# bentotten/radiation_ppo

Measured on AMD Instinct MI355X. Metric: env steps/sec (whole node) at 4096 envs; PPO iters/sec at 1/2/4/8 GPUs, higher is better.
Workload: dtype f32 policy / f64+int32 env

## Files before the change

include/radsearch.h:

```cpp
#ifndef RADSEARCH_H
#define RADSEARCH_H

#include <stddef.h>
#include <stdint.h>

#ifdef __cplusplus
extern "C" {
#endif

#define RS_ABI_VERSION 4
#define RS_OBS_DIM 11
#define RS_NUM_ACTIONS 9
#define RS_MAX_AGENTS 8
#define RS_MAX_OBS 7

typedef void* rs_stream_t;
typedef struct rs_handle rs_handle;

enum {
    RS_OK = 0,
    RS_ERR_INVALID_ARG = 1,
    RS_ERR_HIP = 2,
    RS_ERR_WORKSPACE = 3,
    RS_ERR_UNSUPPORTED = 4
// ... 127 lines not shown
typedef struct rs_update_state {
    int32_t adam_step;
    int32_t stopped;
    int32_t iters;
    int32_t pad;
    double last_stats[5];
} rs_update_state;

int rs_adam_step(const rs_mlp_params* actor, const rs_mlp_params* critic, const float* grads, float* m, float* v,
                 const double* stats, rs_update_state* state, float lr, float kl_threshold, rs_stream_t stream);

int rs_ppo_update_step(const rs_mlp_params* actor, const rs_mlp_params* critic, const rs_ppo_batch* batch, float* grads,
                       double* stats, void* workspace, float* m, float* v, rs_update_state* state, float lr, float kl_threshold,
                       rs_stream_t stream);

typedef struct rs_maps rs_maps;
enum {
    RS_MAPERR_RING_FULL = 1,
    RS_MAPERR_VISIT_OVERFLOW = 2,
    RS_MAPERR_OFF_MAP = 4
};
size_t rs_maps_state_bytes(int32_t num_envs, int32_t num_agents, int32_t steps_per_episode, int32_t map_x, int32_t map_y);
int rs_maps_create(int32_t num_envs, int32_t num_agents, int32_t steps_per_episode, int32_t map_x, int32_t map_y,
                   double resolution_accuracy, const float* visit_table, void* workspace, size_t workspace_bytes,
                   rs_stream_t stream, rs_maps** out);
void rs_maps_destroy(rs_maps* m);
int rs_maps_reset(rs_maps* m, const uint8_t* mask, rs_stream_t stream);
int rs_maps_update(rs_maps* m, rs_handle* env, const float* obs, const float* pred, const uint8_t* mask, rs_stream_t stream);
int rs_maps_stack(rs_maps* m, float* actor_stack, float* critic_stack, rs_stream_t stream);
int rs_maps_field(rs_maps* m, const char* name, void** dev_ptr, int32_t* elem_bytes, int32_t* rows, int32_t* cols);
// ... 274 lines not shown
```

radiation_ppo_amd/_lib.py:

```python
import ctypes as C
import os

import torch

_PKG = os.path.dirname(os.path.abspath(__file__))
LIB_PATH = os.environ.get("RS_LIB_PATH") or os.path.join(_PKG, "lib", "librs_hip.so")

RS_OBS_DIM = 11
RS_MAX_AGENTS = 8
RS_MAX_OBS = 7

ENVERR_ZERO_DIST = 1
ENVERR_IDLE_STALL = 2
ENVERR_CORRECT_CAP = 4
ENVERR_BAD_ACTION = 8
ENVERR_NO_PATH = 16

MAPERR_RING_FULL = 1
MAPERR_VISIT_OVERFLOW = 2
MAPERR_OFF_MAP = 4


class RsConfig(C.Structure):
    _fields_ = [
# ... 78 lines not shown
                                   C.c_void_p, C.c_void_p, C.c_void_p]),
    ("rs_error_flags", C.c_int, [C.c_void_p, C.c_void_p, C.POINTER(C.c_uint32)]),
    ("rs_policy_forward", C.c_int, [C.POINTER(RsMlpParams), C.POINTER(RsMlpParams), C.c_void_p, C.c_int32, C.c_void_p,
                                    C.c_void_p, C.c_void_p]),
    ("rs_ff_team_step", C.c_int, [C.POINTER(RsMlpParams), C.POINTER(RsMlpParams), C.c_int32, C.c_void_p, C.c_void_p, C.c_void_p,
                                  C.c_void_p, C.c_void_p, C.c_void_p, C.c_int32, C.c_void_p]),
    ("rs_rollout", C.c_int, [C.c_void_p, C.POINTER(RsMlpParams), C.POINTER(RsMlpParams), C.POINTER(RsRolloutArgs), C.c_void_p]),
    ("rs_rollout_lds_bytes", C.c_size_t, [C.c_int]),
    ("rs_ppo_grad_workspace_bytes", C.c_size_t, []),
    ("rs_ppo_grad", C.c_int, [C.POINTER(RsMlpParams), C.POINTER(RsMlpParams), C.POINTER(RsPpoBatch), C.c_void_p, C.c_void_p,
                              C.c_void_p, C.c_void_p, C.c_void_p]),
    ("rs_adam_step", C.c_int, [C.POINTER(RsMlpParams), C.POINTER(RsMlpParams), C.c_void_p, C.c_void_p, C.c_void_p, C.c_void_p,
                               C.c_void_p, C.c_float, C.c_float, C.c_void_p]),
    ("rs_ppo_update_step", C.c_int, [C.POINTER(RsMlpParams), C.POINTER(RsMlpParams), C.POINTER(RsPpoBatch), C.c_void_p, C.c_void_p,
                                     C.c_void_p, C.c_void_p, C.c_void_p, C.c_void_p, C.c_float, C.c_float, C.c_void_p]),
    ("rs_maps_state_bytes", C.c_size_t, [C.c_int32, C.c_int32, C.c_int32, C.c_int32, C.c_int32]),
    ("rs_maps_create", C.c_int, [C.c_int32, C.c_int32, C.c_int32, C.c_int32, C.c_int32, C.c_double, C.c_void_p, C.c_void_p,
                                 C.c_size_t, C.c_void_p, C.POINTER(C.c_void_p)]),
    ("rs_maps_destroy", None, [C.c_void_p]),
    ("rs_maps_reset", C.c_int, [C.c_void_p, C.c_void_p, C.c_void_p]),
    ("rs_maps_update", C.c_int, [C.c_void_p, C.c_void_p, C.c_void_p, C.c_void_p, C.c_void_p, C.c_void_p]),
    ("rs_maps_stack", C.c_int, [C.c_void_p, C.c_void_p, C.c_void_p, C.c_void_p]),
    ("rs_maps_field", C.c_int, [C.c_void_p, C.c_char_p, C.POINTER(C.c_void_p), C.POINTER(C.c_int32), C.POINTER(C.c_int32),
                                C.POINTER(C.c_int32)]),
    ("rs_cnn_trunk_slab_row", C.c_int32, [C.c_int32]),
    ("rs_cnn_trunk_slab_rows", C.c_int32, [C.c_int64, C.c_int32]),
    ("rs_cnn_trunk_forward_grid", C.c_int32, [C.c_int64, C.c_int32]),
    ("rs_cnn_trunk_scratch_floats", C.c_int32, [C.c_int32]),
    ("rs_cnn_trunk_forward", C.c_int, [C.c_void_p, C.c_void_p, C.c_void_p, C.c_int32, C.c_int32, C.c_int64, C.c_void_p, C.c_void_p,
                                       C.c_void_p, C.c_void_p, C.c_void_p, C.c_void_p, C.c_void_p, C.c_void_p, C.c_void_p, C.c_void_p]),
# ... 141 lines not shown
```

radiation_ppo_amd/build.py:

```python
import os
import shutil
import subprocess
import sys
from concurrent.futures import ThreadPoolExecutor

PKG = os.path.dirname(os.path.abspath(__file__))
ROOT = os.path.dirname(PKG)
CSRC = os.path.join(PKG, "csrc")
LIBDIR = os.path.join(PKG, "lib")
OBJDIR = os.path.join(LIBDIR, "obj")
LIB = os.path.join(LIBDIR, "librs_hip.so")

SOURCES = ["rs_env.hip", "rs_ppo.hip", "rs_maps.hip", "rs_cnn.hip", "rs_cnn_sized.hip", "rs_pfgru.hip", "rs_gru.hip", "rs_pfgru_train.hip", "rs_rnn_policy.hip", "rs_welford.hip", "rs_cnn_loss.hip",
           "rs_rnn_sized.hip", "rs_pfgru_sized.hip", "rs_pfgru_sized_train.hip", "rs_ff_team.hip", "rs_eval.hip", "rs_draws.hip", "rs_cnn_eval.hip"]
CFLAGS = ["--offload-arch=gfx950", "-O3", "-std=c++17", "-fPIC", "-ffp-contract=off", "-fno-fast-math", "-Wall",
          "-Wno-unused-function"]
EXTRA_CFLAGS = {"rs_ppo.hip": ["-fno-slp-vectorize"], "rs_ff_team.hip": ["-fno-slp-vectorize"], "rs_eval.hip": ["-fno-slp-vectorize"],
                "rs_rnn_sized.hip": ["-mllvm", "-pragma-unroll-threshold=1000000"],
                "rs_pfgru_sized.hip": ["-mllvm", "-pragma-unroll-threshold=1000000"]}


def hipcc() -> str:
    for c in (os.environ.get("HIPCC"), shutil.which("hipcc"), "/opt/rocm/bin/hipcc"):
        if c and os.path.exists(c):
# ... 35 lines not shown
        cpus = os.cpu_count() or 1
    jobs = max(1, min(len(SOURCES), cpus, int(os.environ.get("MAX_JOBS") or cpus)))
    order = sorted(SOURCES, key=lambda f: f not in ("rs_rnn_sized.hip", "rs_pfgru_sized.hip"))
    with ThreadPoolExecutor(max_workers=jobs) as ex:
        done = dict(zip(order, ex.map(compile_one, order)))
    objs = [done[f] for f in SOURCES]
    cmd = [cc, "--offload-arch=gfx950", "-shared", "-fPIC"] + objs + ["-o", lib]
    if verbose:
        print("[radiation_ppo_amd.build]", " ".join(cmd), flush=True)
    subprocess.run(cmd, check=True)
    return lib


if __name__ == "__main__":
    prio = sys.argv[sys.argv.index("--prio") + 1] if "--prio" in sys.argv else None
    if "--stamps" in sys.argv:
        build(force="--force" in sys.argv, defines=["RS_K7_STAMPS"], suffix="_stamps")
    elif "--skew" in sys.argv or prio is not None:
        skew = "--skew" in sys.argv
        build(force="--force" in sys.argv, defines=(["RS_K7_SKEW"] if skew else []) + ([f"RS_K7_PRIO={int(prio)}"] if prio is not None else []),
              suffix=("_skew" if skew else "") + (f"_prio{int(prio)}" if prio is not None else ""))
    else:
        build(force="--force" in sys.argv)
```

radiation_ppo_amd/csrc/rs_ppo.hip:

```cpp
#include <hip/hip_runtime.h>
#include <stdint.h>
#include <stdlib.h>
#include <string.h>

#include "../../include/radsearch.h"
#include "rs_mlp.hpp"
#include "rs_handle.hpp"

static inline RsMlpParams to_dev(const rs_mlp_params* p) { return RsMlpParams{p->w1, p->b1, p->w2, p->b2, p->w3, p->b3}; }

__device__ __forceinline__ void rs_exchange_x(const float (&xo)[RS_IN_PAD], float (&xp)[RS_IN_PAD]) {
#pragma unroll
    for (int k = 0; k < RS_IN_PAD; ++k) xp[k] = __shfl_xor(xo[k], 32);
}

__global__ void __launch_bounds__(64) rs_policy_forward_kernel(RsMlpParams pa, RsMlpParams pc, const float* __restrict__ x, int M,
                                                               float* __restrict__ logits, float* __restrict__ value) {
    extern __shared__ __align__(16) float smem_f[];
    RsMlpLds<8> A; RsMlpLds<1> Cn;
    A.carve(smem_f);
    Cn.carve(smem_f + rs_mlp_lds_floats(8));
    A.fill(pa); Cn.fill(pc);
    __syncthreads();
    const int lane = threadIdx.x & 63;
// ... 265 lines not shown

struct RsGradWs { float *pa, *pc; double *sa, *sc; int* snap; };

static RsGradWs rs_grad_ws(void* workspace) {
    const int slabs = RS_GRAD_BLOCKS;
    RsGradWs w;
    w.pa = static_cast<float*>(workspace);
    w.pc = w.pa + (size_t)slabs * rs_net_params(8);
    w.sa = reinterpret_cast<double*>((reinterpret_cast<uintptr_t>(w.pc + (size_t)slabs * rs_net_params(1)) + 255) & ~uintptr_t(255));
    w.sc = w.sa + (size_t)slabs * 5;
    w.snap = reinterpret_cast<int*>(w.sc + (size_t)slabs * 5);
    return w;
}

static int rs_launch_k7(const rs_mlp_params* actor, const rs_mlp_params* critic, const rs_ppo_batch* batch, const RsGradWs& w,
                        const int32_t* stop_flag, const rs_update_state* ust, hipStream_t s, bool pair = false) {
    const size_t lds_a = sizeof(float) * (size_t)rs_grad2_lds_floats(8);
    const size_t lds_c = sizeof(float) * (size_t)rs_grad2_lds_floats(1);
    const size_t lds_p = lds_a > lds_c ? lds_a : lds_c;
    if (pair) {
        if (hipFuncSetAttribute(reinterpret_cast<const void*>(rs_ppo_grad2_pair_kernel), hipFuncAttributeMaxDynamicSharedMemorySize, (int)lds_p) != hipSuccess)
            return RS_ERR_HIP;
    } else if (hipFuncSetAttribute(reinterpret_cast<const void*>(rs_ppo_grad2_kernel<8>), hipFuncAttributeMaxDynamicSharedMemorySize, (int)lds_a) != hipSuccess ||
               hipFuncSetAttribute(reinterpret_cast<const void*>(rs_ppo_grad2_kernel<1>), hipFuncAttributeMaxDynamicSharedMemorySize, (int)lds_c) != hipSuccess)
        return RS_ERR_HIP;
    int threads = 512;
#if defined(RS_K7_STAMPS) || defined(RS_K7_SKEW)
    if (const char* e = getenv("RS_K7_THREADS")) threads = atoi(e) == 256 ? 256 : 512;
#endif
    if (pair) {
        hipLaunchKernelGGL(rs_ppo_grad2_pair_kernel, dim3(2 * RS_GRAD_BLOCKS), dim3(threads), lds_p, s, to_dev(actor), to_dev(critic), *batch,
                           w.pa, w.pc, w.sa, w.sc, stop_flag, ust, ust ? w.snap : (int*)nullptr);
        return RS_OK;
    }
    hipLaunchKernelGGL(rs_ppo_grad2_kernel<8>, dim3(RS_GRAD_BLOCKS), dim3(threads), lds_a, s, to_dev(actor), *batch, w.pa, w.sa, stop_flag,
                       (const rs_update_state*)nullptr, (int*)nullptr);
    hipLaunchKernelGGL(rs_ppo_grad2_kernel<1>, dim3(RS_GRAD_BLOCKS), dim3(threads), lds_c, s, to_dev(critic), *batch, w.pc, w.sc, stop_flag,
                       ust, ust ? w.snap : (int*)nullptr);
    return RS_OK;
}

int rs_ppo_grad(const rs_mlp_params* actor, const rs_mlp_params* critic, const rs_ppo_batch* batch, float* grads,
                double* stats, void* workspace, const int32_t* stop_flag, rs_stream_t stream) {
    if (!actor || !critic || !batch || !grads || !stats || !workspace || batch->M < 1) return RS_ERR_INVALID_ARG;
    if (reinterpret_cast<uintptr_t>(workspace) & 255u) return RS_ERR_WORKSPACE;
    hipStream_t s = static_cast<hipStream_t>(stream);
    const RsGradWs w = rs_grad_ws(workspace);
    if (const int rc = rs_launch_k7(actor, critic, batch, w, stop_flag, nullptr, s)) return rc;
    const int np = rs_net_params(8) + rs_net_params(1);
    hipLaunchKernelGGL(rs_ppo_reduce_kernel, dim3((np + 63) / 64), dim3(1024), 0, s, w.pa, w.pc, w.sa, w.sc, RS_GRAD_BLOCKS, grads, stats,
                       batch->alpha, batch->vf_coef, stop_flag);
    return hipGetLastError() == hipSuccess ? RS_OK : RS_ERR_HIP;
}

int rs_ppo_update_step(const rs_mlp_params* actor, const rs_mlp_params* critic, const rs_ppo_batch* batch, float* grads,
                       double* stats, void* workspace, float* m, float* v, rs_update_state* state, float lr, float kl_threshold,
                       rs_stream_t stream) {
    if (!actor || !critic || !batch || !grads || !stats || !workspace || !m || !v || !state || batch->M < 1) return RS_ERR_INVALID_ARG;
    if (reinterpret_cast<uintptr_t>(workspace) & 255u) return RS_ERR_WORKSPACE;
    hipStream_t s = static_cast<hipStream_t>(stream);
    const RsGradWs w = rs_grad_ws(workspace);
    const char* split = getenv("RS_PPO_SPLIT_GRAD");
    if (const int rc = rs_launch_k7(actor, critic, batch, w, &state->stopped, state, s, !(split && *split && *split != '0'))) return rc;
    const int np = rs_net_params(8) + rs_net_params(1);
    hipLaunchKernelGGL(rs_ppo_tail_kernel, dim3((np + 63) / 64), dim3(1024), 0, s, w.pa, w.pc, w.sa, w.sc, RS_GRAD_BLOCKS, grads, stats,
                       batch->alpha, batch->vf_coef, rs_param_seg(actor, critic), m, v, state, w.snap, lr, kl_threshold);
    return hipGetLastError() == hipSuccess ? RS_OK : RS_ERR_HIP;
}

#ifdef RS_K7_STAMPS
int rs_debug_k7_stamps(unsigned long long* out, int clear) {
    if (hipDeviceSynchronize() != hipSuccess) return RS_ERR_HIP;
    if (out && hipMemcpyFromSymbol(out, HIP_SYMBOL(rs_k7_stamp_table), sizeof(unsigned long long) * 2 * RS_K7_NPH) != hipSuccess) return RS_ERR_HIP;
    if (clear) {
        unsigned long long z[2 * RS_K7_NPH] = {0};
        if (hipMemcpyToSymbol(HIP_SYMBOL(rs_k7_stamp_table), z, sizeof(z)) != hipSuccess) return RS_ERR_HIP;
    }
    return RS_OK;
}
#endif

#ifdef RS_K7_SKEW
// ... 36 lines not shown
```

radiation_ppo_amd/csrc/rs_ppo_grad2.hpp:

```cpp
#pragma once
#include "rs_mlp.hpp"

#define RS_T2 33

#ifdef RS_K7_STAMPS
#define RS_K7_NPH 16
__device__ unsigned long long rs_k7_stamp_table[2][RS_K7_NPH];
#define RS_STAMP_ENTRY const unsigned long long st_rt0 = __builtin_amdgcn_s_memrealtime(); const unsigned long long st_t0 = rs_k7_now();
#define RS_STAMP_DECL unsigned long long st_acc[RS_K7_NPH] = {0}; unsigned long long st_last = rs_k7_now(); st_acc[12] = st_last - st_t0;
#define RS_STAMP_EXIT(net) do { RS_STAMP(13); if ((threadIdx.x & 63) == 0) { st_acc[14] = __builtin_amdgcn_s_memrealtime() - st_rt0; \
                           for (int q = 0; q < RS_K7_NPH; ++q) atomicAdd(&rs_k7_stamp_table[net][q], st_acc[q]); } } while (0)
#define RS_STAMP(i) do { __builtin_amdgcn_sched_barrier(0); asm volatile("; RS_STAMP_MARK " #i); const unsigned long long t_ = rs_k7_now(); st_acc[i] += t_ - st_last; st_last = t_; \
                         __builtin_amdgcn_sched_barrier(0); } while (0)
__device__ __forceinline__ unsigned long long rs_k7_now() {
    unsigned long long t;
    asm volatile("s_memtime %0\n\ts_waitcnt lgkmcnt(0)" : "=s"(t) :: "memory");
    return t;
}
#else
#define RS_STAMP_ENTRY
#define RS_STAMP_DECL
#define RS_STAMP_EXIT(net)
#ifdef RS_K7_NO_PHASE_FENCE
#define RS_STAMP(i) do {} while (0)
// ... 31 lines not shown
#define RS_SKEW_RELEASED
#define RS_SKEW_PAIRS(net, slots)
#define RS_SKEW_EXIT(net)
#endif

#ifndef RS_K7_PRIO
#define RS_K7_PRIO 1
#endif
#ifndef RS_K7_PRIO_BIT
#define RS_K7_PRIO_BIT 15
#endif
#define RS_K7_PROG_FLOATS 8

#define RS_XRAW 400
#define RS_XSC 192
#define RS_G2_WAVE_FLOATS ((64 + 32) * RS_T2 + RS_XRAW + RS_XSC + 64)

__host__ __device__ constexpr int rs_grad2_lds_floats(int nout) {
    return ((rs_mlp_lds_floats(nout) + 3) & ~3) + 2 * 2 * 16 * 64 + 2 * 4 * 64 + 8 * RS_G2_WAVE_FLOATS + RS_K7_PROG_FLOATS + RS_SKEW_LDS_FLOATS;
}

__device__ __forceinline__ float rs_other_half(float x, int h) {
    const auto r = __builtin_amdgcn_permlane32_swap(__float_as_uint(x), __float_as_uint(x), false, false);
    return __uint_as_float(h ? r[0] : r[1]);
}

typedef float rs_f2 __attribute__((ext_vector_type(2)));

__device__ __forceinline__ void rs_tanh_scaled16(f32x16& v) {
#pragma unroll
    for (int r = 0; r < 16; r += 2) {
        const rs_f2 e = (rs_f2){1.0f, 1.0f} + (rs_f2){__builtin_amdgcn_exp2f(v[r]), __builtin_amdgcn_exp2f(v[r + 1])};
        const rs_f2 t = __builtin_elementwise_fma((rs_f2){-2.0f, -2.0f}, (rs_f2){__builtin_amdgcn_rcpf(e.x), __builtin_amdgcn_rcpf(e.y)},
                                                  (rs_f2){1.0f, 1.0f});
        v[r] = t.x; v[r + 1] = t.y;
    }
}

__device__ __forceinline__ rs_f2 rs_dtanh2(rs_f2 d, rs_f2 hv) { return __builtin_elementwise_fma(-(d * hv), hv, d); }

__device__ __forceinline__ void rs_stage32(float* T, const f32x16& v, int c, int h) {
#pragma unroll
    for (int r = 0; r < 16; ++r) T[rs_kappa(r, h) * RS_T2 + c] = v[r];
}

template <int NOUT>
__device__ __forceinline__ void rs_ppo_grad2_body(const RsMlpParams prm, const rs_ppo_batch B, float* partial,
                                                  double* stat_partial, const int* stop,
                                                  const rs_update_state* ust, int* snap,
                                                  const int bid, const int nblocks) {
    extern __shared__ __align__(16) float smem_f[];
    if (snap && bid == 0 && threadIdx.x == 0) { snap[0] = ust->adam_step; snap[1] = ust->stopped; }
    if (stop && *stop) return;
    RS_STAMP_ENTRY
    RS_SKEW_ENTRY
    RsMlpLds<NOUT> W;
    W.carve(smem_f);
    float* w2tf = smem_f + ((rs_mlp_lds_floats(NOUT) + 3) & ~3);
    float* w3tf = w2tf + 2 * 2 * 16 * 64;
    const int wid = __builtin_amdgcn_readfirstlane(threadIdx.x >> 6);
    const int lane = threadIdx.x & 63, h = lane >> 5, c = lane & 31;
    const int l15 = lane & 15, l4 = lane >> 4;
    float* Qt = w3tf + 2 * 4 * 64 + wid * RS_G2_WAVE_FLOATS;
    float* Pt = Qt + 64 * RS_T2;
    float* xraw = Pt + 32 * RS_T2;
// ... 42 lines not shown
#pragma unroll
        for (int r = 0; r < 16; ++r) { acc2[a][0][r] = 0.f; acc2[a][1][r] = 0.f; }
#pragma unroll
    for (int r = 0; r < 4; ++r) {
#pragma unroll
        for (int a = 0; a < 4; ++a) acc1[a][r] = 0.f;
        acc3[0][r] = 0.f; acc3[1][r] = 0.f;
    }
    f32x4 accs;
#pragma unroll
    for (int r = 0; r < 4; ++r) accs[r] = 0.f;

    const int trips = (groups + n_waves - 1) / n_waves;
    const long x_last = (long)M * RS_IN - 1;
    auto dma_rows = [&](int g) {
        const char* gx = reinterpret_cast<const char*>(B.x + (long)g * (32 * RS_IN));
        const int lim = (int)(x_last - (long)g * (32 * RS_IN));
#pragma unroll
        for (int i = 0; i < 6; ++i) {
            const int o = min(i * 64 + lane, lim);
            __builtin_amdgcn_global_load_lds((const __attribute__((address_space(1))) void*)(gx + 4u * (unsigned)o),
                                             (__attribute__((address_space(3))) void*)(xraw + i * 64), 4, 0, 0);
        }
    };
    auto dma_scal = [&](int g) {
        const int m0 = g * 32;
        const int ms = min(m0 + c, M - 1);
        if constexpr (NOUT == 8) {
            const int mi = min(m0 + (lane >> 1), M - 1);
            const int* src = reinterpret_cast<const int*>(B.act) + 2 * (size_t)mi + (lane & 1);
            __builtin_amdgcn_global_load_lds((const __attribute__((address_space(1))) void*)src,
                                             (__attribute__((address_space(3))) void*)(xsc), 4, 0, 0);
        }
        if constexpr (NOUT == 8) {
            const float* src = (h ? B.logp_old : B.adv) + ms;
            __builtin_amdgcn_global_load_lds((const __attribute__((address_space(1))) void*)src,
                                             (__attribute__((address_space(3))) void*)(xsc + 64), 4, 0, 0);
        }
        {
            const float* src = (h ? B.ret : B.w) + ms;
// ... 25 lines not shown
        const int bit = (int)(__builtin_amdgcn_readfirstlane((int)(__builtin_amdgcn_s_memtime() >> RS_K7_PRIO_BIT)) & 1) ^ (wid >> 2);
        if (bit) __builtin_amdgcn_s_setprio(1);
        else __builtin_amdgcn_s_setprio(0);
#endif
    };
#if RS_K7_PRIO == 4
    if (wid >= 4) __builtin_amdgcn_s_setprio(1);
#endif
    RS_STAMP_DECL
    for (int trip = 0; trip < trips; ++trip) {
        RS_STAMP(15);
        balance(RS_K7_PRIO == 2 ? 2 * trip : trip);
        const int gi_raw = wave_g + trip * n_waves;
        const int gi = gi_raw < groups ? gi_raw : groups - 1;
        const int m = gi * 32 + c;
        const bool valid = gi_raw < groups && m < M;
        asm volatile("s_waitcnt vmcnt(0)" ::: "memory");
#if defined(RS_K7_ALIGN) && RS_K7_ALIGN >= 1
        __builtin_amdgcn_s_barrier();
#endif
        const float wi = valid ? xsc[128 + c] : 0.0f;
        const int s_act = reinterpret_cast<const int*>(xsc)[2 * c];
        const float s_adv = xsc[64 + c], s_lpo = xsc[96 + c], s_ret = xsc[160 + c];
        float xv[6];
#pragma unroll
        for (int s6 = 0; s6 < 6; ++s6) xv[s6] = xraw[c * RS_IN + 2 * s6 + h];
        if (h) xv[5] = 1.0f;
        RS_STAMP(0);
        f32x16 H1[2], H2[2];
#pragma unroll
        for (int it = 0; it < 2; ++it)
#pragma unroll
            for (int r = 0; r < 16; ++r) H1[it][r] = 0.0f;
        {
            float a0 = w1b[(0 * 6 + 0) * 64 + lane], a1 = w1b[(1 * 6 + 0) * 64 + lane];
#pragma unroll
            for (int s = 0; s < 6; ++s) {
                const float b = xv[s];
                float n0 = 0.f, n1 = 0.f;
                if (s + 1 < 6) { n0 = w1b[(0 * 6 + s + 1) * 64 + lane]; n1 = w1b[(1 * 6 + s + 1) * 64 + lane]; }
                H1[0] = __builtin_amdgcn_mfma_f32_32x32x2f32(a0, b, H1[0], 0, 0, 0);
                H1[1] = __builtin_amdgcn_mfma_f32_32x32x2f32(a1, b, H1[1], 0, 0, 0);
// ... 187 lines not shown
                    acc3[hf] = __builtin_amdgcn_mfma_f32_4x4x1f32(av[q].z, bv[q].z, acc3[hf], 0, 0, 0);
                    accs = __builtin_amdgcn_mfma_f32_4x4x1f32(z1, 1.0f, accs, 0, 0, 0);
                    acc3[hf] = __builtin_amdgcn_mfma_f32_4x4x1f32(av[q].w, bv[q].w, acc3[hf], 0, 0, 0);
                }
            }
        }
        RS_STAMP(7);
        if (NOUT == 8) {
#pragma unroll
            for (int it = 0; it < 2; ++it) {
                f32x16 t;
#pragma unroll
                for (int r = 0; r < 16; ++r) t[r] = 0.f;
#pragma unroll
                for (int s = 0; s < 4; ++s) {
                    const float b = h ? dz[(2 * s + 1) % NOUT] : dz[(2 * s) % NOUT];
                    t = __builtin_amdgcn_mfma_f32_32x32x2f32(w3tf[(it * 4 + s) * 64 + lane], b, t, 0, 0, 0);
                }
#pragma unroll
                for (int r = 0; r < 16; r += 2) {
                    const rs_f2 d = rs_dtanh2((rs_f2){t[r], t[r + 1]}, (rs_f2){H2[it][r], H2[it][r + 1]});
                    H2[it][r] = d.x; H2[it][r + 1] = d.y;
                }
            }
        } else {
#pragma unroll
            for (int kt = 0; kt < 2; ++kt)
#pragma unroll
                for (int r = 0; r < 16; r += 2) {
                    const rs_f2 d = (rs_f2){w3v[kt * 16 + r], w3v[kt * 16 + r + 1]} * (rs_f2){dz[0], dz[0]};
                    const rs_f2 e = rs_dtanh2(d, (rs_f2){H2[kt][r], H2[kt][r + 1]});
// ... 29 lines not shown
                    n0 = wq[((0 * 2 + ((g4 + 1) >> 2)) * 4 + ((g4 + 1) & 3)) * 64];
                    n1 = wq[((1 * 2 + ((g4 + 1) >> 2)) * 4 + ((g4 + 1) & 3)) * 64];
                }
                D1[0] = __builtin_amdgcn_mfma_f32_32x32x2f32(a0.x, H2[kt][r0 + 0], D1[0], 0, 0, 0);
                D1[1] = __builtin_amdgcn_mfma_f32_32x32x2f32(a1.x, H2[kt][r0 + 0], D1[1], 0, 0, 0);
                D1[0] = __builtin_amdgcn_mfma_f32_32x32x2f32(a0.y, H2[kt][r0 + 1], D1[0], 0, 0, 0);
                D1[1] = __builtin_amdgcn_mfma_f32_32x32x2f32(a1.y, H2[kt][r0 + 1], D1[1], 0, 0, 0);
                D1[0] = __builtin_amdgcn_mfma_f32_32x32x2f32(a0.z, H2[kt][r0 + 2], D1[0], 0, 0, 0);
                D1[1] = __builtin_amdgcn_mfma_f32_32x32x2f32(a1.z, H2[kt][r0 + 2], D1[1], 0, 0, 0);
                D1[0] = __builtin_amdgcn_mfma_f32_32x32x2f32(a0.w, H2[kt][r0 + 3], D1[0], 0, 0, 0);
                D1[1] = __builtin_amdgcn_mfma_f32_32x32x2f32(a1.w, H2[kt][r0 + 3], D1[1], 0, 0, 0);
                a0 = n0; a1 = n1;
            }
        }
        float xb[8];
        {
            int gi_late = gi;
            asm volatile("" : "+v"(gi_late));
#pragma unroll
            for (int s8 = 0; s8 < 8; ++s8) {
                int n = gi_late * 32 + 4 * s8 + l4;
                n = n < M ? n : M - 1;
                xb[s8] = (l15 < RS_IN) ? B.x[(size_t)n * RS_IN + l15] : ((l15 == RS_IN) ? 1.0f : 0.0f);
            }
        }
#pragma unroll
        for (int it = 0; it < 2; ++it)
#pragma unroll
            for (int r = 0; r < 16; r += 2) {
                const rs_f2 hv = {Qt[(32 * it + rs_kappa(r, h)) * RS_T2 + c], Qt[(32 * it + rs_kappa(r + 1, h)) * RS_T2 + c]};
                const rs_f2 d = rs_dtanh2((rs_f2){D1[it][r], D1[it][r + 1]}, hv);
// ... 144 lines not shown
template <int NOUT>
__global__ void __launch_bounds__(512, 2) rs_ppo_grad2_kernel(RsMlpParams prm, rs_ppo_batch B, float* __restrict__ partial,
                                                              double* __restrict__ stat_partial, const int* __restrict__ stop,
                                                              const rs_update_state* __restrict__ ust, int* __restrict__ snap) {
    rs_ppo_grad2_body<NOUT>(prm, B, partial, stat_partial, stop, ust, snap, blockIdx.x, gridDim.x);
}

__global__ void __launch_bounds__(512, 2) rs_ppo_grad2_pair_kernel(RsMlpParams pa, RsMlpParams pc, rs_ppo_batch B, float* __restrict__ partial_a,
                                                                   float* __restrict__ partial_c, double* __restrict__ stat_a,
                                                                   double* __restrict__ stat_c, const int* __restrict__ stop,
                                                                   const rs_update_state* __restrict__ ust, int* __restrict__ snap) {
    const int G = gridDim.x >> 1;
    if ((int)blockIdx.x < G) rs_ppo_grad2_body<8>(pa, B, partial_a, stat_a, stop, nullptr, nullptr, blockIdx.x, G);
    else rs_ppo_grad2_body<1>(pc, B, partial_c, stat_c, stop, ust, snap, blockIdx.x - G, G);
}
```

radiation_ppo_amd/ppo.py:

```python
import ctypes as C
import os
from dataclasses import dataclass
from typing import Any, Dict, List, Optional

import torch
import torch.distributed as dist
import torch.nn as nn

from . import _lib
from .envs import RadSearchVec, gae as rs_gae_call


class FFActorCritic(nn.Module):

    def __init__(self, state_dim: int = 11, action_dim: int = 8, hidden: int = 64):
        super().__init__()
        self.actor = nn.Sequential(nn.Linear(state_dim, hidden), nn.Tanh(), nn.Linear(hidden, hidden), nn.Tanh(),
                                   nn.Linear(hidden, action_dim), nn.Softmax(dim=-1))
        self.critic = nn.Sequential(nn.Linear(state_dim, hidden), nn.Tanh(), nn.Linear(hidden, hidden), nn.Tanh(),
                                    nn.Linear(hidden, 1))

    def logits(self, x: torch.Tensor) -> torch.Tensor:
        for layer in list(self.actor)[:-1]:
            x = layer(x)
# ... 48 lines not shown
        self.lib = _lib.load()
        self.ac = ac
        dev = next(ac.parameters()).device
        self.bucket = torch.zeros(N_PARAMS + 16, dtype=torch.float32, device=dev)
        self.grads = self.bucket[:N_PARAMS]
        self.stats = torch.zeros(5, dtype=torch.float64, device=dev)
        self.stats_from_bucket = False
        self.ws = torch.empty(self.lib.rs_ppo_grad_workspace_bytes() + 256, dtype=torch.uint8, device=dev)
        self._ws_ptr = self.ws.data_ptr() + (-self.ws.data_ptr()) % 256
        order = [ac.actor[0].weight, ac.actor[0].bias, ac.actor[2].weight, ac.actor[2].bias, ac.actor[4].weight, ac.actor[4].bias,
                 ac.critic[0].weight, ac.critic[0].bias, ac.critic[2].weight, ac.critic[2].bias, ac.critic[4].weight, ac.critic[4].bias]
        self.m = torch.zeros(N_PARAMS, dtype=torch.float32, device=dev)
        self.v = torch.zeros(N_PARAMS, dtype=torch.float32, device=dev)
        self.state = torch.zeros(8, dtype=torch.float64, device=dev)
        self.state_i32 = self.state.view(torch.int32)
        self.views = []
        o = 0
        for p in order:
            self.views.append((p, self.grads[o:o + p.numel()].view_as(p)))
            o += p.numel()
        assert o == N_PARAMS

    def begin_update(self) -> None:
        self.state_i32[1:3].zero_()

    def adam_step(self, lr: float, kl_threshold: float) -> None:
        import ctypes as C
        pa, pc = mlp_params(self.ac.actor), mlp_params(self.ac.critic)
        _lib.check(self.lib.rs_adam_step(C.byref(pa), C.byref(pc), self.bucket.data_ptr(), self.m.data_ptr(), self.v.data_ptr(),
                                         None if self.stats_from_bucket else self.stats.data_ptr(), self.state.data_ptr(), lr, kl_threshold,
# ... 17 lines not shown
        with _lib.timed("rs_ppo_grad"):
            _lib.check(self.lib.rs_ppo_grad(C.byref(pa), C.byref(pc), C.byref(b), self.bucket.data_ptr(), self.stats.data_ptr(),
                                            self._ws_ptr, (self.state.data_ptr() + 4) if use_stop_flag else None,
                                            torch.cuda.current_stream(X.device).cuda_stream), "rs_ppo_grad")
        return self.stats, self.grads

    def bind(self, X, act, adv, ret, logp_old, w, clip_ratio: float, alpha: float, vf_coef: float = 0.01) -> None:
        import ctypes as C
        for t in (X, adv, ret, logp_old, w):
            assert t.dtype == torch.float32 and t.is_contiguous()
        assert act.dtype == torch.int64 and act.is_contiguous()
        b = _lib.RsPpoBatch(X.data_ptr(), act.data_ptr(), adv.data_ptr(), ret.data_ptr(), logp_old.data_ptr(), w.data_ptr(),
                            X.shape[0], clip_ratio, alpha, vf_coef)
        pa, pc = mlp_params(self.ac.actor), mlp_params(self.ac.critic)
        self._bound = (b, pa, pc, (X, act, adv, ret, logp_old, w))
        self._bound_args = (C.byref(pa), C.byref(pc), C.byref(b), self.bucket.data_ptr(), self.stats.data_ptr(), self._ws_ptr,
                            self.m.data_ptr(), self.v.data_ptr(), self.state.data_ptr())
        self._bound_dev = X.device

    def step_bound(self, lr: float, kl_threshold: float):
        self.stats_from_bucket = False
        with _lib.timed("rs_ppo_grad"):
            _lib.check(self.lib.rs_ppo_update_step(*self._bound_args, lr, kl_threshold,
                                                   torch.cuda.current_stream(self._bound_dev).cuda_stream), "rs_ppo_update_step")
        return self.stats, self.grads

    def step(self, X, act, adv, ret, logp_old, w, clip_ratio: float, alpha: float, vf_coef: float = 0.01, *, lr: float,
             kl_threshold: float):
        self.bind(X, act, adv, ret, logp_old, w, clip_ratio, alpha, vf_coef)
        return self.step_bound(lr, kl_threshold)

    def allreduce(self) -> None:
        Collectives.all_reduce_sum(self.bucket)
        self.stats_from_bucket = True

    def assign_grads(self) -> None:
        for p, g in self.views:
            p.grad = g

# ... 279 lines not shown
            else:
                kl_reached = True
            kk += 1
        self.pi_scheduler.step()
        return UpdateResult(stop_iteration=kk, loss_policy=last[4], loss_critic=last[3], loss_predictor=0.0,
                            kl_divergence=last[0], Entropy=last[1], ClipFrac=last[2], LocLoss=0.0)

    def _update_agent_fused(self, X, act, adv, ret, logp_old, w) -> UpdateResult:
        if self._fused is None:
            self._fused = FusedPPOGrad(self.agent)
        f = self._fused
        lr = self.actor_learning_rate * (0.99 ** (self.epochs_done // 100))
        thr = 1.5 * self.target_kl
        f.begin_update()
        one_rank = _world() == 1 and not os.environ.get("RS_PPO_SPLIT_TAIL")
        if one_rank:
            f.bind(X, act, adv, ret, logp_old, w, self.clip_ratio, self.alpha)
        for _ in range(self.train_pi_iters):
            if one_rank:
                f.step_bound(lr, thr)
                continue
            stats, grads = f(X, act, adv, ret, logp_old, w, self.clip_ratio, self.alpha, use_stop_flag=True)
            if _world() > 1:
                f.allreduce()
            f.adam_step(lr, thr)
        kk, stopped, _, last = f.read_state()
        self.epochs_done += 1
        return UpdateResult(stop_iteration=kk, loss_policy=last[4], loss_critic=last[3], loss_predictor=0.0,
                            kl_divergence=last[0], Entropy=last[1], ClipFrac=last[2], LocLoss=0.0)

    def save(self, path: str) -> None:
        torch.save(self.agent.state_dict(), path)

    def load(self, path: str) -> None:
        self.agent.load_state_dict(torch.load(path, map_location=self.device, weights_only=True))

    def resume_state(self) -> Dict[str, Any]:
# ... 480 lines not shown
```

Measured before the change: 44.93 million.

## Prebuild swizzled PPO batch image once per update for direct LDS DMA loads

Adds a kernel that repacks the PPO batch (observations, actions, advantages, returns, logp, weights) into a per-32-row record laid out in the exact lane order the gradient kernel consumes. The gradient kernels get image variants that load these records with whole-wave global_load_lds DMA pieces and float4 loads, in place of per-row strided gathers with bounds clamping. The image is built once per bind and reused across all train_pi_iters. The multi-rank path now also binds once instead of rebuilding args every iteration. The cost is an extra buffer and a build kernel per update, plus a compile-time parts mask that selects which sections use the image.

```diff
diff --git a/include/radsearch.h b/include/radsearch.h
--- a/include/radsearch.h
+++ b/include/radsearch.h
@@ -165,6 +165,14 @@
                        double* stats, void* workspace, float* m, float* v, rs_update_state* state, float lr, float kl_threshold,
                        rs_stream_t stream);
 
+size_t rs_ppo_batch_image_bytes(int32_t M);
+int rs_ppo_batch_image_build(const rs_ppo_batch* batch, void* image, rs_stream_t stream);
+int rs_ppo_grad_img(const rs_mlp_params* actor, const rs_mlp_params* critic, const rs_ppo_batch* batch, const void* image, float* grads,
+                    double* stats, void* workspace, const int32_t* stop_flag, rs_stream_t stream);
+int rs_ppo_update_step_img(const rs_mlp_params* actor, const rs_mlp_params* critic, const rs_ppo_batch* batch, const void* image,
+                           float* grads, double* stats, void* workspace, float* m, float* v, rs_update_state* state, float lr,
+                           float kl_threshold, rs_stream_t stream);
+
 typedef struct rs_maps rs_maps;
 enum {
     RS_MAPERR_RING_FULL = 1,
diff --git a/radiation_ppo_amd/_lib.py b/radiation_ppo_amd/_lib.py
--- a/radiation_ppo_amd/_lib.py
+++ b/radiation_ppo_amd/_lib.py
@@ -116,6 +116,12 @@
                                C.c_void_p, C.c_float, C.c_float, C.c_void_p]),
     ("rs_ppo_update_step", C.c_int, [C.POINTER(RsMlpParams), C.POINTER(RsMlpParams), C.POINTER(RsPpoBatch), C.c_void_p, C.c_void_p,
                                      C.c_void_p, C.c_void_p, C.c_void_p, C.c_void_p, C.c_float, C.c_float, C.c_void_p]),
+    ("rs_ppo_batch_image_bytes", C.c_size_t, [C.c_int32]),
+    ("rs_ppo_batch_image_build", C.c_int, [C.POINTER(RsPpoBatch), C.c_void_p, C.c_void_p]),
+    ("rs_ppo_grad_img", C.c_int, [C.POINTER(RsMlpParams), C.POINTER(RsMlpParams), C.POINTER(RsPpoBatch), C.c_void_p, C.c_void_p, C.c_void_p,
+                                  C.c_void_p, C.c_void_p, C.c_void_p]),
+    ("rs_ppo_update_step_img", C.c_int, [C.POINTER(RsMlpParams), C.POINTER(RsMlpParams), C.POINTER(RsPpoBatch), C.c_void_p, C.c_void_p,
+                                         C.c_void_p, C.c_void_p, C.c_void_p, C.c_void_p, C.c_void_p, C.c_float, C.c_float, C.c_void_p]),
     ("rs_maps_state_bytes", C.c_size_t, [C.c_int32, C.c_int32, C.c_int32, C.c_int32, C.c_int32]),
     ("rs_maps_create", C.c_int, [C.c_int32, C.c_int32, C.c_int32, C.c_int32, C.c_int32, C.c_double, C.c_void_p, C.c_void_p,
                                  C.c_size_t, C.c_void_p, C.POINTER(C.c_void_p)]),
diff --git a/radiation_ppo_amd/build.py b/radiation_ppo_amd/build.py
--- a/radiation_ppo_amd/build.py
+++ b/radiation_ppo_amd/build.py
@@ -73,7 +73,12 @@
 
 if __name__ == "__main__":
     prio = sys.argv[sys.argv.index("--prio") + 1] if "--prio" in sys.argv else None
-    if "--stamps" in sys.argv:
+    parts = sys.argv[sys.argv.index("--img-parts") + 1] if "--img-parts" in sys.argv else None
+    if parts is not None:
+        st = "--stamps" in sys.argv
+        build(force="--force" in sys.argv, defines=(["RS_K7_STAMPS"] if st else []) + [f"RS_K7_IMG_PARTS={int(parts)}"],
+              suffix=("_stamps" if st else "") + f"_img{int(parts)}")
+    elif "--stamps" in sys.argv:
         build(force="--force" in sys.argv, defines=["RS_K7_STAMPS"], suffix="_stamps")
     elif "--skew" in sys.argv or prio is not None:
         skew = "--skew" in sys.argv
diff --git a/radiation_ppo_amd/csrc/rs_ppo.hip b/radiation_ppo_amd/csrc/rs_ppo.hip
--- a/radiation_ppo_amd/csrc/rs_ppo.hip
+++ b/radiation_ppo_amd/csrc/rs_ppo.hip
@@ -303,11 +303,18 @@
 }
 
 static int rs_launch_k7(const rs_mlp_params* actor, const rs_mlp_params* critic, const rs_ppo_batch* batch, const RsGradWs& w,
-                        const int32_t* stop_flag, const rs_update_state* ust, hipStream_t s, bool pair = false) {
+                        const int32_t* stop_flag, const rs_update_state* ust, hipStream_t s, bool pair = false, const float* img = nullptr) {
     const size_t lds_a = sizeof(float) * (size_t)rs_grad2_lds_floats(8);
     const size_t lds_c = sizeof(float) * (size_t)rs_grad2_lds_floats(1);
     const size_t lds_p = lds_a > lds_c ? lds_a : lds_c;
-    if (pair) {
+    if (img) {
+        if (pair) {
+            if (hipFuncSetAttribute(reinterpret_cast<const void*>(rs_ppo_grad2_img_pair_kernel), hipFuncAttributeMaxDynamicSharedMemorySize, (int)lds_p) != hipSuccess)
+                return RS_ERR_HIP;
+        } else if (hipFuncSetAttribute(reinterpret_cast<const void*>(rs_ppo_grad2_img_kernel<8>), hipFuncAttributeMaxDynamicSharedMemorySize, (int)lds_a) != hipSuccess ||
+                   hipFuncSetAttribute(reinterpret_cast<const void*>(rs_ppo_grad2_img_kernel<1>), hipFuncAttributeMaxDynamicSharedMemorySize, (int)lds_c) != hipSuccess)
+            return RS_ERR_HIP;
+    } else if (pair) {
         if (hipFuncSetAttribute(reinterpret_cast<const void*>(rs_ppo_grad2_pair_kernel), hipFuncAttributeMaxDynamicSharedMemorySize, (int)lds_p) != hipSuccess)
             return RS_ERR_HIP;
     } else if (hipFuncSetAttribute(reinterpret_cast<const void*>(rs_ppo_grad2_kernel<8>), hipFuncAttributeMaxDynamicSharedMemorySize, (int)lds_a) != hipSuccess ||
@@ -317,6 +324,19 @@
 #if defined(RS_K7_STAMPS) || defined(RS_K7_SKEW)
     if (const char* e = getenv("RS_K7_THREADS")) threads = atoi(e) == 256 ? 256 : 512;
 #endif
+    int* const snap = ust ? w.snap : (int*)nullptr;
+    if (img) {
+        if (pair) {
+            hipLaunchKernelGGL(rs_ppo_grad2_img_pair_kernel, dim3(2 * RS_GRAD_BLOCKS), dim3(threads), lds_p, s, to_dev(actor), to_dev(critic), *batch,
+                               img, w.pa, w.pc, w.sa, w.sc, stop_flag, ust, snap);
+            return RS_OK;
+        }
+        hipLaunchKernelGGL(rs_ppo_grad2_img_kernel<8>, dim3(RS_GRAD_BLOCKS), dim3(threads), lds_a, s, to_dev(actor), *batch, img, w.pa, w.sa,
+                           stop_flag, (const rs_update_state*)nullptr, (int*)nullptr);
+        hipLaunchKernelGGL(rs_ppo_grad2_img_kernel<1>, dim3(RS_GRAD_BLOCKS), dim3(threads), lds_c, s, to_dev(critic), *batch, img, w.pc, w.sc,
+                           stop_flag, ust, snap);
+        return RS_OK;
+    }
     if (pair) {
         hipLaunchKernelGGL(rs_ppo_grad2_pair_kernel, dim3(2 * RS_GRAD_BLOCKS), dim3(threads), lds_p, s, to_dev(actor), to_dev(critic), *batch,
                            w.pa, w.pc, w.sa, w.sc, stop_flag, ust, ust ? w.snap : (int*)nullptr);
@@ -329,32 +349,70 @@
     return RS_OK;
 }
 
-int rs_ppo_grad(const rs_mlp_params* actor, const rs_mlp_params* critic, const rs_ppo_batch* batch, float* grads,
-                double* stats, void* workspace, const int32_t* stop_flag, rs_stream_t stream) {
+size_t rs_ppo_batch_image_bytes(int32_t M) {
+    return M < 1 ? 0 : (size_t)((M + 31) / 32) * RS_IMG_REC * sizeof(float);
+}
+
+int rs_ppo_batch_image_build(const rs_ppo_batch* batch, void* image, rs_stream_t stream) {
+    if (!batch || !image || batch->M < 1 || !batch->x || !batch->act || !batch->adv || !batch->ret || !batch->logp_old || !batch->w)
+        return RS_ERR_INVALID_ARG;
+    if (reinterpret_cast<uintptr_t>(image) & 15u) return RS_ERR_INVALID_ARG;
+    hipLaunchKernelGGL(rs_ppo_batch_image_kernel, dim3((batch->M + 31) / 32), dim3(256), 0, static_cast<hipStream_t>(stream), *batch,
+                       static_cast<float*>(image));
+    return hipGetLastError() == hipSuccess ? RS_OK : RS_ERR_HIP;
+}
+
+static int rs_ppo_grad_on(const rs_mlp_params* actor, const rs_mlp_params* critic, const rs_ppo_batch* batch, const float* image, float* grads,
+                          double* stats, void* workspace, const int32_t* stop_flag, rs_stream_t stream) {
     if (!actor || !critic || !batch || !grads || !stats || !workspace || batch->M < 1) return RS_ERR_INVALID_ARG;
     if (reinterpret_cast<uintptr_t>(workspace) & 255u) return RS_ERR_WORKSPACE;
     hipStream_t s = static_cast<hipStream_t>(stream);
     const RsGradWs w = rs_grad_ws(workspace);
-    if (const int rc = rs_launch_k7(actor, critic, batch, w, stop_flag, nullptr, s)) return rc;
+    if (const int rc = rs_launch_k7(actor, critic, batch, w, stop_flag, nullptr, s, false, image)) return rc;
     const int np = rs_net_params(8) + rs_net_params(1);
     hipLaunchKernelGGL(rs_ppo_reduce_kernel, dim3((np + 63) / 64), dim3(1024), 0, s, w.pa, w.pc, w.sa, w.sc, RS_GRAD_BLOCKS, grads, stats,
                        batch->alpha, batch->vf_coef, stop_flag);
     return hipGetLastError() == hipSuccess ? RS_OK : RS_ERR_HIP;
 }
 
-int rs_ppo_update_step(const rs_mlp_params* actor, const rs_mlp_params* critic, const rs_ppo_batch* batch, float* grads,
-                       double* stats, void* workspace, float* m, float* v, rs_update_state* state, float lr, float kl_threshold,
-                       rs_stream_t stream) {
+int rs_ppo_grad(const rs_mlp_params* actor, const rs_mlp_params* critic, const rs_ppo_batch* batch, float* grads,
+                double* stats, void* workspace, const int32_t* stop_flag, rs_stream_t stream) {
+    return rs_ppo_grad_on(actor, critic, batch, nullptr, grads, stats, workspace, stop_flag, stream);
+}
+
+int rs_ppo_grad_img(const rs_mlp_params* actor, const rs_mlp_params* critic, const rs_ppo_batch* batch, const void* image, float* grads,
+                    double* stats, void* workspace, const int32_t* stop_flag, rs_stream_t stream) {
+    if (!image || (reinterpret_cast<uintptr_t>(image) & 15u)) return RS_ERR_INVALID_ARG;
+    return rs_ppo_grad_on(actor, critic, batch, static_cast<const float*>(image), grads, stats, workspace, stop_flag, stream);
+}
+
+static int rs_ppo_update_step_on(const rs_mlp_params* actor, const rs_mlp_params* critic, const rs_ppo_batch* batch, const float* image,
+                                 float* grads, double* stats, void* workspace, float* m, float* v, rs_update_state* state, float lr,
+                                 float kl_threshold, rs_stream_t stream) {
     if (!actor || !critic || !batch || !grads || !stats || !workspace || !m || !v || !state || batch->M < 1) return RS_ERR_INVALID_ARG;
     if (reinterpret_cast<uintptr_t>(workspace) & 255u) return RS_ERR_WORKSPACE;
     hipStream_t s = static_cast<hipStream_t>(stream);
     const RsGradWs w = rs_grad_ws(workspace);
     const char* split = getenv("RS_PPO_SPLIT_GRAD");
-    if (const int rc = rs_launch_k7(actor, critic, batch, w, &state->stopped, state, s, !(split && *split && *split != '0'))) return rc;
+    if (const int rc = rs_launch_k7(actor, critic, batch, w, &state->stopped, state, s, !(split && *split && *split != '0'), image)) return rc;
     const int np = rs_net_params(8) + rs_net_params(1);
     hipLaunchKernelGGL(rs_ppo_tail_kernel, dim3((np + 63) / 64), dim3(1024), 0, s, w.pa, w.pc, w.sa, w.sc, RS_GRAD_BLOCKS, grads, stats,
                        batch->alpha, batch->vf_coef, rs_param_seg(actor, critic), m, v, state, w.snap, lr, kl_threshold);
     return hipGetLastError() == hipSuccess ? RS_OK : RS_ERR_HIP;
+}
+
+int rs_ppo_update_step(const rs_mlp_params* actor, const rs_mlp_params* critic, const rs_ppo_batch* batch, float* grads,
+                       double* stats, void* workspace, float* m, float* v, rs_update_state* state, float lr, float kl_threshold,
+                       rs_stream_t stream) {
+    return rs_ppo_update_step_on(actor, critic, batch, nullptr, grads, stats, workspace, m, v, state, lr, kl_threshold, stream);
+}
+
+int rs_ppo_update_step_img(const rs_mlp_params* actor, const rs_mlp_params* critic, const rs_ppo_batch* batch, const void* image, float* grads,
+                           double* stats, void* workspace, float* m, float* v, rs_update_state* state, float lr, float kl_threshold,
+                           rs_stream_t stream) {
+    if (!image || (reinterpret_cast<uintptr_t>(image) & 15u)) return RS_ERR_INVALID_ARG;
+    return rs_ppo_update_step_on(actor, critic, batch, static_cast<const float*>(image), grads, stats, workspace, m, v, state, lr, kl_threshold,
+                                 stream);
 }
 
 #ifdef RS_K7_STAMPS
diff --git a/radiation_ppo_amd/csrc/rs_ppo_grad2.hpp b/radiation_ppo_amd/csrc/rs_ppo_grad2.hpp
--- a/radiation_ppo_amd/csrc/rs_ppo_grad2.hpp
+++ b/radiation_ppo_amd/csrc/rs_ppo_grad2.hpp
@@ -69,6 +69,19 @@
 
 #define RS_XRAW 400
 #define RS_XSC 192
+
+#define RS_IMG_A 0
+#define RS_IMG_S 384
+#define RS_IMG_B 576
+#define RS_IMG_REC 1088
+#ifndef RS_K7_IMG_PARTS
+#define RS_K7_IMG_PARTS 7
+#endif
+
+template <int OFF>
+__device__ __forceinline__ void rs_dma_piece(const float* g, float* l) {
+    __builtin_amdgcn_global_load_lds((const __attribute__((address_space(1))) void*)g, (__attribute__((address_space(3))) void*)l, 4, OFF, 0);
+}
 #define RS_G2_WAVE_FLOATS ((64 + 32) * RS_T2 + RS_XRAW + RS_XSC + 64)
 
 __host__ __device__ constexpr int rs_grad2_lds_floats(int nout) {
@@ -99,11 +112,12 @@
     for (int r = 0; r < 16; ++r) T[rs_kappa(r, h) * RS_T2 + c] = v[r];
 }
 
-template <int NOUT>
+template <int NOUT, bool IMG = false>
 __device__ __forceinline__ void rs_ppo_grad2_body(const RsMlpParams prm, const rs_ppo_batch B, float* partial,
                                                   double* stat_partial, const int* stop,
                                                   const rs_update_state* ust, int* snap,
-                                                  const int bid, const int nblocks) {
+                                                  const int bid, const int nblocks, const float* img = nullptr) {
+    constexpr bool IA = IMG && (RS_K7_IMG_PARTS & 1), IB = IMG && (RS_K7_IMG_PARTS & 2), IS = IMG && (RS_K7_IMG_PARTS & 4);
     extern __shared__ __align__(16) float smem_f[];
     if (snap && bid == 0 && threadIdx.x == 0) { snap[0] = ust->adam_step; snap[1] = ust->stopped; }
     if (stop && *stop) return;
@@ -176,6 +190,14 @@
     const int trips = (groups + n_waves - 1) / n_waves;
     const long x_last = (long)M * RS_IN - 1;
     auto dma_rows = [&](int g) {
+        if constexpr (IA) {
+            const float* rec = img + (long)g * RS_IMG_REC + RS_IMG_A;
+            asm volatile("" : "+s"(rec));
+            const float* src = rec + (unsigned)lane;
+            rs_dma_piece<0>(src, xraw); rs_dma_piece<256>(src, xraw); rs_dma_piece<512>(src, xraw);
+            rs_dma_piece<768>(src, xraw); rs_dma_piece<1024>(src, xraw); rs_dma_piece<1280>(src, xraw);
+            return;
+        }
         const char* gx = reinterpret_cast<const char*>(B.x + (long)g * (32 * RS_IN));
         const int lim = (int)(x_last - (long)g * (32 * RS_IN));
 #pragma unroll
@@ -186,6 +208,14 @@
         }
     };
     auto dma_scal = [&](int g) {
+        if constexpr (IS) {
+            const float* rec = img + (long)g * RS_IMG_REC + RS_IMG_S;
+            asm volatile("" : "+s"(rec));
+            const float* src = rec + (unsigned)lane;
+            if constexpr (NOUT == 8) { rs_dma_piece<0>(src, xsc); rs_dma_piece<256>(src, xsc); }
+            rs_dma_piece<512>(src, xsc);
+            return;
+        }
         const int m0 = g * 32;
         const int ms = min(m0 + c, M - 1);
         if constexpr (NOUT == 8) {
@@ -241,18 +271,18 @@
         const int gi_raw = wave_g + trip * n_waves;
         const int gi = gi_raw < groups ? gi_raw : groups - 1;
         const int m = gi * 32 + c;
-        const bool valid = gi_raw < groups && m < M;
+        const bool valid = gi_raw < groups && (IS || m < M);
         asm volatile("s_waitcnt vmcnt(0)" ::: "memory");
 #if defined(RS_K7_ALIGN) && RS_K7_ALIGN >= 1
         __builtin_amdgcn_s_barrier();
 #endif
         const float wi = valid ? xsc[128 + c] : 0.0f;
-        const int s_act = reinterpret_cast<const int*>(xsc)[2 * c];
+        const int s_act = reinterpret_cast<const int*>(xsc)[IS ? c : 2 * c];
         const float s_adv = xsc[64 + c], s_lpo = xsc[96 + c], s_ret = xsc[160 + c];
         float xv[6];
 #pragma unroll
-        for (int s6 = 0; s6 < 6; ++s6) xv[s6] = xraw[c * RS_IN + 2 * s6 + h];
-        if (h) xv[5] = 1.0f;
+        for (int s6 = 0; s6 < 6; ++s6) xv[s6] = IA ? xraw[64 * s6 + lane] : xraw[c * RS_IN + 2 * s6 + h];
+        if (!IA && h) xv[5] = 1.0f;
         RS_STAMP(0);
         f32x16 H1[2], H2[2];
 #pragma unroll
@@ -470,7 +500,8 @@
                 for (int r = 0; r < 16; ++r) t[r] = 0.f;
 #pragma unroll
                 for (int s = 0; s < 4; ++s) {
-                    const float b = h ? dz[(2 * s + 1) % NOUT] : dz[(2 * s) % NOUT];
+                    const float dz_lo = dz[(2 * s) % NOUT], dz_hi = dz[(2 * s + 1) % NOUT];
+                    const float b = h ? dz_hi : dz_lo;
                     t = __builtin_amdgcn_mfma_f32_32x32x2f32(w3tf[(it * 4 + s) * 64 + lane], b, t, 0, 0, 0);
                 }
 #pragma unroll
@@ -530,7 +561,16 @@
             }
         }
         float xb[8];
-        {
+        if constexpr (IB) {
+            int gi_late = gi;
+            asm volatile("" : "+s"(gi_late));
+            const float* rec = img + (long)gi_late * RS_IMG_REC + RS_IMG_B;
+            asm volatile("" : "+s"(rec));
+            const float4* pb = reinterpret_cast<const float4*>(rec) + (unsigned)lane;
+            const float4 b0 = pb[0], b1 = pb[64];
+            xb[0] = b0.x; xb[1] = b0.y; xb[2] = b0.z; xb[3] = b0.w;
+            xb[4] = b1.x; xb[5] = b1.y; xb[6] = b1.z; xb[7] = b1.w;
+        } else {
             int gi_late = gi;
             asm volatile("" : "+v"(gi_late));
 #pragma unroll
@@ -705,3 +745,45 @@
     if ((int)blockIdx.x < G) rs_ppo_grad2_body<8>(pa, B, partial_a, stat_a, stop, nullptr, nullptr, blockIdx.x, G);
     else rs_ppo_grad2_body<1>(pc, B, partial_c, stat_c, stop, ust, snap, blockIdx.x - G, G);
 }
+
+template <int NOUT>
+__global__ void __launch_bounds__(512, 2) rs_ppo_grad2_img_kernel(RsMlpParams prm, rs_ppo_batch B, const float* __restrict__ img,
+                                                                  float* __restrict__ partial, double* __restrict__ stat_partial,
+                                                                  const int* __restrict__ stop, const rs_update_state* __restrict__ ust,
+                                                                  int* __restrict__ snap) {
+    rs_ppo_grad2_body<NOUT, true>(prm, B, partial, stat_partial, stop, ust, snap, blockIdx.x, gridDim.x, img);
+}
+
+__global__ void __launch_bounds__(512, 2) rs_ppo_grad2_img_pair_kernel(RsMlpParams pa, RsMlpParams pc, rs_ppo_batch B, const float* __restrict__ img,
+                                                                       float* __restrict__ partial_a, float* __restrict__ partial_c,
+                                                                       double* __restrict__ stat_a, double* __restrict__ stat_c,
+                                                                       const int* __restrict__ stop, const rs_update_state* __restrict__ ust,
+                                                                       int* __restrict__ snap) {
+    const int G = gridDim.x >> 1;
+    if ((int)blockIdx.x < G) rs_ppo_grad2_body<8, true>(pa, B, partial_a, stat_a, stop, nullptr, nullptr, blockIdx.x, G, img);
+    else rs_ppo_grad2_body<1, true>(pc, B, partial_c, stat_c, stop, ust, snap, blockIdx.x - G, G, img);
+}
+
+__global__ void __launch_bounds__(256) rs_ppo_batch_image_kernel(rs_ppo_batch B, float* __restrict__ img) {
+    const long g = blockIdx.x;
+    const long M = B.M;
+    float* rec = img + g * RS_IMG_REC;
+    for (int i = threadIdx.x; i < RS_IMG_REC; i += 256) {
+        float v;
+        if (i < RS_IMG_S) {
+            const int l = i & 63, k = 2 * (i >> 6) + (l >> 5);
+            const long e = g * (32 * RS_IN) + (l & 31) * RS_IN + k;
+            v = k < RS_IN ? B.x[e < M * RS_IN ? e : M * RS_IN - 1] : 1.0f;
+        } else if (i < RS_IMG_B) {
+            const int j = i - RS_IMG_S, row = j >> 5;
+            const long m = g * 32 + (j & 31), mc = m < M ? m : M - 1;
+            v = row == 0 ? __int_as_float((int)B.act[mc]) : row == 1 ? 0.0f : row == 2 ? B.adv[mc] : row == 3 ? B.logp_old[mc]
+              : row == 4 ? (m < M ? B.w[m] : 0.0f) : B.ret[mc];
+        } else {
+            const int j = i - RS_IMG_B, l = (j >> 2) & 63, l15 = l & 15, s8 = 4 * (j >> 8) + (j & 3);
+            const long n = g * 32 + 4 * s8 + (l >> 4), nc = n < M ? n : M - 1;
+            v = l15 < RS_IN ? B.x[nc * RS_IN + l15] : (l15 == RS_IN ? 1.0f : 0.0f);
+        }
+        rec[i] = v;
+    }
+}
diff --git a/radiation_ppo_amd/ppo.py b/radiation_ppo_amd/ppo.py
--- a/radiation_ppo_amd/ppo.py
+++ b/radiation_ppo_amd/ppo.py
@@ -86,6 +86,8 @@
         self.v = torch.zeros(N_PARAMS, dtype=torch.float32, device=dev)
         self.state = torch.zeros(8, dtype=torch.float64, device=dev)
         self.state_i32 = self.state.view(torch.int32)
+        self.image = None
+        self._bound = None
         self.views = []
         o = 0
         for p in order:
@@ -133,15 +135,36 @@
                             X.shape[0], clip_ratio, alpha, vf_coef)
         pa, pc = mlp_params(self.ac.actor), mlp_params(self.ac.critic)
         self._bound = (b, pa, pc, (X, act, adv, ret, logp_old, w))
-        self._bound_args = (C.byref(pa), C.byref(pc), C.byref(b), self.bucket.data_ptr(), self.stats.data_ptr(), self._ws_ptr,
-                            self.m.data_ptr(), self.v.data_ptr(), self.state.data_ptr())
         self._bound_dev = X.device
+        stream = torch.cuda.current_stream(X.device).cuda_stream
+        self._bound_img = None
+        if not os.environ.get("RS_PPO_NO_IMAGE"):
+            need = self.lib.rs_ppo_batch_image_bytes(X.shape[0])
+            if self.image is None or self.image.numel() < need:
+                self.image = None
+                self.image = torch.empty(need, dtype=torch.uint8, device=X.device)
+            assert self.image.data_ptr() % 16 == 0
+            _lib.check(self.lib.rs_ppo_batch_image_build(C.byref(b), self.image.data_ptr(), stream), "rs_ppo_batch_image_build")
+            self._bound_img = self.image.data_ptr()
+        head = (C.byref(pa), C.byref(pc), C.byref(b)) + (() if self._bound_img is None else (self._bound_img,))
+        self._bound_args = head + (self.bucket.data_ptr(), self.stats.data_ptr(), self._ws_ptr,
+                                   self.m.data_ptr(), self.v.data_ptr(), self.state.data_ptr())
+        self._bound_grad_args = head + (self.bucket.data_ptr(), self.stats.data_ptr(), self._ws_ptr)
+        self._bound_step = self.lib.rs_ppo_update_step if self._bound_img is None else self.lib.rs_ppo_update_step_img
+        self._bound_grad = self.lib.rs_ppo_grad if self._bound_img is None else self.lib.rs_ppo_grad_img
 
     def step_bound(self, lr: float, kl_threshold: float):
         self.stats_from_bucket = False
         with _lib.timed("rs_ppo_grad"):
-            _lib.check(self.lib.rs_ppo_update_step(*self._bound_args, lr, kl_threshold,
-                                                   torch.cuda.current_stream(self._bound_dev).cuda_stream), "rs_ppo_update_step")
+            _lib.check(self._bound_step(*self._bound_args, lr, kl_threshold,
+                                        torch.cuda.current_stream(self._bound_dev).cuda_stream), "rs_ppo_update_step")
+        return self.stats, self.grads
+
+    def grad_bound(self, use_stop_flag: bool = False):
+        self.stats_from_bucket = False
+        with _lib.timed("rs_ppo_grad"):
+            _lib.check(self._bound_grad(*self._bound_grad_args, (self.state.data_ptr() + 4) if use_stop_flag else None,
+                                        torch.cuda.current_stream(self._bound_dev).cuda_stream), "rs_ppo_grad")
         return self.stats, self.grads
 
     def step(self, X, act, adv, ret, logp_old, w, clip_ratio: float, alpha: float, vf_coef: float = 0.01, *, lr: float,
@@ -451,13 +474,12 @@
         thr = 1.5 * self.target_kl
         f.begin_update()
         one_rank = _world() == 1 and not os.environ.get("RS_PPO_SPLIT_TAIL")
-        if one_rank:
-            f.bind(X, act, adv, ret, logp_old, w, self.clip_ratio, self.alpha)
+        f.bind(X, act, adv, ret, logp_old, w, self.clip_ratio, self.alpha)
         for _ in range(self.train_pi_iters):
             if one_rank:
                 f.step_bound(lr, thr)
                 continue
-            stats, grads = f(X, act, adv, ret, logp_old, w, self.clip_ratio, self.alpha, use_stop_flag=True)
+            stats, grads = f.grad_bound(use_stop_flag=True)
             if _world() > 1:
                 f.allreduce()
             f.adam_step(lr, thr)
```

New measurement: 45.37 million (median of 6 runs). No clear change (+1.0%).
